# Banksylel/Restrictive-Hierarchical-Semantic-Segmentation

Measured on AMD Instinct MI355X. Metric: train images/sec (620x620, hier-HRNet-W48), higher is better.
Workload: dtype f32 (fp16x2 split on fp16 MFMA, 22-bit operands, fp32 accumulate; exact-fp32 MFMA on the small problems); 1 GPU; HRNet-W48 hierarchical (class_tree_tl.json), 620x620, batch 4 per GPU, train_epoch batch body (fwd L passes, prediction prep + metrics, CE+Dice+consistency, bwd, grad all-reduce, AdamW, metric vectors, one D2H readback of loss+metrics); global_batch=4, parallelism=dp1, launch=launch tape replay, rccl_ranks=1, level_passes=batched (one launch per layer for all L passes)

## Files before the change

restrictive-hierarchical-semantic-segmentation_amd/csrc/conv.hip:

```cpp
#include "conv_common.h"

static bool igemm_overridden() { return hrseg_g_igemm_wtm || hrseg_g_igemm_kc || hrseg_g_igemm_db || hrseg_g_igemm_ksplit; }

__global__ void zero_f32_kernel(float* __restrict__ p, size_t n) {
  for (size_t i = (size_t)blockIdx.x * blockDim.x + threadIdx.x; i < n; i += (size_t)gridDim.x * blockDim.x) p[i] = 0.f;
}
static void zero_f32(float* p, size_t n, hipStream_t st) {
  size_t blocks = (n + 255) / 256;
  if (blocks > 2048) blocks = 2048;
  hipLaunchKernelGGL(zero_f32_kernel, dim3((unsigned)blocks), dim3(256), 0, st, p, n);
}

static IgemmPlan plan_igemm(const IgemmArgs& a) {
  IgemmPlan pl;
  pl.wtn = (a.N % 48 == 0) ? 3 : (a.N % 64 == 0) ? 4 : (a.N % 32 == 0) ? 2 : 1;
  const int kc_max = (a.K % 48 == 0) ? 3 : (a.K % 32 == 0) ? 2 : 1;
  const int ntn = a.N / (16 * pl.wtn);
  const long blocks128 = (long)ceil_div(a.M, 128) * ntn;
  const bool large = blocks128 >= 384;
  pl.wtm = large ? 2 : 1;
  pl.kc = large ? 1 : kc_max;
  pl.db = 1;
  pl.ksplit = 1;
  const long blocks = (long)ceil_div(a.M, 64 * pl.wtm) * ntn;
// ... 550 lines not shown
    if (check_wgrad_span(a[i])) return 1;
    g.gx[i] = gx;
    end += gx * tiles;
    g.blk_end[i] = end;
    g.a[i] = a[i];
  }
  if (sp) {
    hrseg_count(CNT_WGRAD_SP_GROUP);
    return launch_wgrad_group_sp(g, tn, tk, end, st);
  }
  hrseg_count(CNT_WGRAD_F32_GROUP);
  return launch_wgrad_group_f32(g, tn, tk, end, st);
}

static int wgrad9_tnk(const hrseg_conv_shape_t& s) {
  if (!hrseg_g_wgrad9 || s.ksize != 3 || s.stride != 1 || sp_pieces(s.precision) == 0) return 0;
  if (s.Cin % 48 == 0 && s.Cout % 48 == 0) return 3;
  if (s.Cin % 64 == 0 && s.Cout % 64 == 0) return 4;
  return 0;
}
static const int WG9_TARGET[5] = {256, 256, 128, 128, 96};
static void wgrad9_plan(const hrseg_conv_shape_t& s, int tnk, Wgrad9Args& a, int group_n) {
  a.B = s.B; a.H = s.Hi; a.W = s.Wi; a.Cin = s.Cin; a.Cout = s.Cout; a.ldx = s.ldx; a.lddy = s.ldy;
  a.tiles_x = ceil_div(s.Wi, 16); a.tiles_y = ceil_div(s.Hi, 4);
  a.ntiles = s.B * a.tiles_x * a.tiles_y;
  const int npairs = (s.Cout / (16 * tnk)) * (s.Cin / (16 * tnk));
  const int by_n[5] = {0, hrseg_g_wgrad9_blocks1, hrseg_g_wgrad9_blocks2, hrseg_g_wgrad9_blocks3, hrseg_g_wgrad9_blocks4};
  const int target = (group_n <= 4 && by_n[group_n]) ? by_n[group_n] : hrseg_g_wgrad9_blocks ? hrseg_g_wgrad9_blocks : WG9_TARGET[group_n < 4 ? group_n : 4];
  int chunks = ceil_div(target, npairs);
  if (chunks > a.ntiles) chunks = a.ntiles;
  if (chunks < 1) chunks = 1;
  a.per = ceil_div(a.ntiles, chunks);
  a.nchunks = ceil_div(a.ntiles, a.per);
}
struct Wg9Plan { int tnk; Wgrad9Args a[WG9_MAXG]; };
static bool wgrad9_plan_all(int n, const hrseg_conv_shape_t* shapes, Wg9Plan& pl) {
  if (n < 1 || n > WG9_MAXG) return false;
  pl.tnk = wgrad9_tnk(shapes[0]);
  if (!pl.tnk) return false;
  for (int i = 0; i < n; ++i) {
    if (wgrad9_tnk(shapes[i]) != pl.tnk || shapes[i].precision != shapes[0].precision) return false;
    wgrad9_plan(shapes[i], pl.tnk, pl.a[i], n);
  }
  return true;
}
static size_t wgrad9_ws_bytes(int n, const hrseg_conv_shape_t* shapes) {
  Wg9Plan pl;
// ... 224 lines not shown
      c.Ho = hc; c.Wo = wc; c.M = s->B * hc * wc;
      c.oys = c.oxs = 2; c.oy0 = py; c.ox0 = px;
      pack_taps(c, n, oy, ox, wtp);
      cls[ncls++] = c;
    }
  if (ncls >= 2) {
    const int rc = launch_group_checked(cls, ncls, s->precision, st, "igemm_group(dgrad s2)");
    if (rc <= 0) return rc;
  }
  for (int i = 0; i < ncls; ++i) {
    if (int e = dispatch_igemm(cls[i], s->precision, st)) return e;
    HRSEG_LAUNCH_CHECK("igemm_conv(dgrad s2)");
  }
  return 0;
}

static int wgrad_one(const float* x, const float* dy, float* dw, const hrseg_conv_shape_t* s_in, hipStream_t st,
                     const char* who) {
  hrseg_conv_shape_t sh;
  resolve_wgrad_shapes(1, s_in, &sh);
  const hrseg_conv_shape_t* s = &sh;
  HRSEG_CHECK_ARG(x && dy && dw, "%s: null pointer", who);
  if (s->Cin <= HRSEG_SMALL_CIN_MAX) {
    const long M = (long)s->B * s->Ho * s->Wo;
    const int nblk_target = hrseg_g_deterministic ? 1 : hrseg_g_wgrad_blocks ? hrseg_g_wgrad_blocks : 512;
    int ppb = (int)ceil_div(ceil_div(M, nblk_target), 64) * 64;
    launch_small_cin_wgrad(x, dy, dw, s, ppb, st);
    hrseg_count(CNT_SMALL_CIN);
    HRSEG_LAUNCH_CHECK("conv_small_cin_wgrad");
    return 0;
  }
  HRSEG_CHECK_ARG(s->Cin % 16 == 0 && s->Cout % 16 == 0, "%s: channels (%d,%d) must be multiples of 16", who, s->Cin, s->Cout);
  HRSEG_CHECK_ARG(s->ldx % 4 == 0 && s->ldy % 4 == 0, "%s: ld must be a multiple of 4", who);
  WgradArgs a;
  fill_wgrad_args(a, x, dy, dw, s);
  if (const int ns = sp_pieces(s->precision)) {
    if (int e = dispatch_wgrad_sp(ns, a, st)) return e;
    HRSEG_LAUNCH_CHECK("wgrad_sp");
    return 0;
  }
  const int tn = (s->Cout % 48 == 0) ? 3 : (s->Cout % 64 == 0) ? 4 : (s->Cout % 32 == 0) ? 2 : 1;
  const int tk = (s->Cin % 48 == 0) ? 3 : (s->Cin % 64 == 0) ? 4 : (s->Cin % 32 == 0) ? 2 : 1;
  const int tiles = (a.Cout / (16 * tn)) * (a.Cin / (16 * tk)) * a.T;
  const int pix = hrseg_g_wgrad_pix ? hrseg_g_wgrad_pix : 64, db = hrseg_g_wgrad_db ? hrseg_g_wgrad_db : 1;
  const int target = hrseg_g_wgrad_blocks ? hrseg_g_wgrad_blocks : wgrad_target_blocks(tiles);
  if (int e = launch_wgrad_f32(a, tn, tk, pix, db, target, st)) return e;
  hrseg_count(CNT_WGRAD_F32);
  HRSEG_LAUNCH_CHECK("wgrad");
  return 0;
}
// ... 137 lines not shown
```

restrictive-hierarchical-semantic-segmentation_amd/csrc/conv_common.h:

```cpp
#pragma once
#include "common.h"

struct IgemmArgs {
  const float* x;
  const float* w;
  const float* bias;
  float* y;
  int ldx, ldy;
  int B, Hi, Wi, K;
  int Ho, Wo, N;
  int M;
  int sy, sx;
  int Hy, Wy, oys, oxs, oy0, ox0;
  int ntaps;
  unsigned long long offy_pk, offx_pk, wtap_pk;
  int T;
  int accumulate;
  float rcp_hw, rcp_w;
  int direct_out;
  const float* xmax;
  float wscale, wscale_inv;
  int oy_min, ox_min;
  const unsigned char* wimg;
  int cv_w1, cv_nb;
// ... 73 lines not shown
struct WeightImageGroup {
  int n;
  int ns;
  int blk_end[MAXG];
  int kind[MAXG];
  int K[MAXG];
  float wscale[MAXG];
  const float* w[MAXG];
  unsigned char* img[MAXG];
};
struct WeightImageTabEntry {
  const float* w;
  unsigned char* img;
  int K, kind, ns, blk_end;
  float wscale;
  int pad;
};

struct Wgrad9Args {
  const float* x; const float* dy; float* ws;
  const float* dymax;
  int ldx, lddy, B, H, W, Cin, Cout;
  int tiles_x, tiles_y, ntiles, nchunks, per;
  int exp_nosplit;
  int x_presplit;
};
#define WG9_MAXG 8
struct Wgrad9Group {
  int n;
  int blk_end[WG9_MAXG];
  Wgrad9Args a[WG9_MAXG];
};
struct Wgrad9Reduce {
  int n;
  int blk_end[WG9_MAXG];
  const float* ws[WG9_MAXG];
  float* dw[WG9_MAXG];
  int nchunks[WG9_MAXG];
  long n4[WG9_MAXG];
};

int launch_igemm_f32(const IgemmArgs& a, const IgemmPlan& pl, hipStream_t st);
int launch_igemm_group_f32(const IgemmGroup& g, int wtm, int wtn, int kc, hipStream_t st);
int launch_wgrad_f32(const WgradArgs& a, int tn, int tk, int pix, int db, int target, hipStream_t st);
int launch_wgrad_group_f32(const WgradGroup& g, int tn, int tk, int nblocks, hipStream_t st);
int launch_sp_kernel(int ns, const IgemmArgs& a, const SpPlan& pl, hipStream_t st);
int launch_spw_kernel(const IgemmArgs& a, int wtn, int ksplit, unsigned char* img, hipStream_t st, bool two_slab_ok);
int launch_sp_group_kernel(int ns, const IgemmGroup& g, int wtm, int wtn, bool full, hipStream_t st);
int launch_patch_sp_kernel(int ns, const IgemmArgs& a, int wtn, int cs, int flip, int blocks, int ntotal, hipStream_t st);
int launch_sp_pgroup_kernel(int ns, const IgemmGroup& g, int wtm, int wtn, int cs, int flip, hipStream_t st);
int launch_ws_kernel(const IgemmArgs& a, int kind, int flip, int blocks, int ntotal, hipStream_t st, int ns = 4);
int launch_ws_group_kernel(const IgemmGroup& g, int flip, hipStream_t st, int ns = 4);
int launch_weight_images(const WeightImageGroup& g, int nblocks, hipStream_t st);
int launch_weight_image_table(const WeightImageTabEntry* tab, int n, int nblocks, hipStream_t st);
int launch_wgrad_sp_kernel(int ns, const WgradArgs& a, int tn, int tk, int gx, int tiles, hipStream_t st);
int launch_wgrad_group_sp(const WgradGroup& g, int tn, int tk, int nblocks, hipStream_t st);
int launch_wgrad_spw_kernel(const WgradArgs& a, int nwc, int gx, int tiles, hipStream_t st);
int launch_wgrad9_kernels(int ns, int tnk, const Wgrad9Group& g, int nblocks, const Wgrad9Reduce& r, int rblocks, hipStream_t st);
int check_wgrad_span(const WgradArgs& a);
#define HRSEG_SMALL_CIN_MAX 8
void launch_small_cin_fwd(const float* x, const float* w, const float* bias, float* y, const hrseg_conv_shape_t* s, hipStream_t st);
void launch_small_cin_wgrad(const float* x, const float* dy, float* dw, const hrseg_conv_shape_t* s, int pix_per_block, hipStream_t st);
void launch_small_cin_dgrad(const float* dy, const float* w, float* dx, int accumulate, const hrseg_conv_shape_t* s, hipStream_t st);

bool scratch_usable();
unsigned char* scratch_reserve(hipStream_t st, size_t bytes);
bool ws_make_images(IgemmArgs* a, const int* kinds, int n, hipStream_t st, int ns);
```

restrictive-hierarchical-semantic-segmentation_amd/csrc/conv_small.hip:

```cpp
#include "conv_common.h"

template <int CMAX>
__global__ __launch_bounds__(256) void conv_small_cin_fwd_kernel(const float* __restrict__ x, int ldx,
                                                                 const float* __restrict__ w,
                                                                 const float* __restrict__ bias,
                                                                 float* __restrict__ y, int ldy, int B, int Hi,
                                                                 int Wi, int Cin, int Ho, int Wo, int Cout,
                                                                 int ks, int stride, const float* __restrict__ res, int ldr,
                                                                 int relu) {
  __shared__ float wl[64 * 9 * CMAX];
  const int T = ks * ks, pad = (ks - 1) / 2;
  const int cb = blockIdx.y * 64;
  for (int i = threadIdx.x; i < 64 * T * Cin; i += 256) {
    const int co = i / (T * Cin);
    wl[i] = (cb + co < Cout) ? w[(size_t)(cb + co) * T * Cin + (i - co * T * Cin)] : 0.f;
  }
  __syncthreads();
  const long M = (long)B * Ho * Wo;
  const long m = (long)blockIdx.x * 64 + (threadIdx.x & 63);
  const int cg = threadIdx.x >> 6;
  if (m >= M) return;
  const int b = (int)(m / ((long)Ho * Wo));
  const int rem = (int)(m - (long)b * Ho * Wo);
  const int oy = rem / Wo, ox = rem - oy * Wo;
// ... 44 lines not shown
    for (int kh = 0; kh < 3; ++kh) {
      const int iy = oy * stride + kh - 1;
      const bool rok = (unsigned)iy < (unsigned)Hi;
#pragma unroll
      for (int kw = 0; kw < 3; ++kw) {
        const int ix = ox * stride + kw - 1;
        const bool ok = rok & ((unsigned)ix < (unsigned)Wi);
        const float* xp = x + ((size_t)(b * Hi + (ok ? iy : 0)) * Wi + (ok ? ix : 0)) * ldx;
#pragma unroll
        for (int ci = 0; ci < 3; ++ci) {
          const float xv = ok ? xp[ci] : 0.f;
#pragma unroll
          for (int j = 0; j < 4; ++j) acc[j] = fmaf(xv, wr[(kh * 3 + kw) * 3 + ci][j], acc[j]);
        }
      }
    }
    f32x4 v = acc + bv;
    if (res) v += *reinterpret_cast<const f32x4*>(res + (size_t)m * ldr + co);
    if (relu) v = relu_nan(v);
    *reinterpret_cast<f32x4*>(y + (size_t)m * ldy + co) = v;
  }
}

__global__ __launch_bounds__(256) void conv_cin3_k3_wgrad_kernel(const float* __restrict__ x, int ldx, const float* __restrict__ dy,
                                                                 int lddy, float* __restrict__ dw, int B, int Hi, int Wi, int Ho,
                                                                 int Wo, int stride, int pix_per_block) {
  constexpr int P = 64;
  __shared__ __attribute__((aligned(16))) float dys[P][64];
  __shared__ __attribute__((aligned(16))) float xs[P][9][4];
  __shared__ float red[3][64][28];
  const int tid = threadIdx.x;
  const int co0 = blockIdx.y * 64, col = tid & 63, pg = tid >> 6;
  const int M = B * Ho * Wo, hw = Ho * Wo;
  const int lo = blockIdx.x * pix_per_block;
  const int hi = min(lo + pix_per_block, M);
  float acc[9][3];
#pragma unroll
  for (int t = 0; t < 9; ++t)
#pragma unroll
    for (int c = 0; c < 3; ++c) acc[t][c] = 0.f;
  for (int s0 = lo; s0 < hi; s0 += P) {
#pragma unroll
    for (int r = 0; r < (P * 16) / 256; ++r) {
      const int j = tid + 256 * r;
      const int pp = j >> 4, c4 = (j & 15) * 4;
      const int m = s0 + pp;
      f32x4 v = {0.f, 0.f, 0.f, 0.f};
      if (m < hi) v = *reinterpret_cast<const f32x4*>(dy + (size_t)m * lddy + co0 + c4);
      *reinterpret_cast<f32x4*>(&dys[pp][c4]) = v;
    }
    for (int j = tid; j < P * 9; j += 256) {
      const int pp = j / 9, t = j - pp * 9;
      const int m = s0 + pp;
      f32x4 v = {0.f, 0.f, 0.f, 0.f};
      if (m < hi) {
        const int b = m / hw, rem = m - b * hw;
        const int oy = rem / Wo, ox = rem - oy * Wo;
        const int iy = oy * stride + t / 3 - 1, ix = ox * stride + t % 3 - 1;
        if ((unsigned)iy < (unsigned)Hi && (unsigned)ix < (unsigned)Wi) {
          const float* xp = x + ((size_t)(b * Hi + iy) * Wi + ix) * ldx;
          v = f32x4{xp[0], xp[1], xp[2], 0.f};
        }
      }
      *reinterpret_cast<f32x4*>(&xs[pp][t][0]) = v;
    }
    __syncthreads();
#pragma unroll 4
    for (int q = 0; q < P / 4; ++q) {
      const int pp = pg * (P / 4) + q;
      const float g = dys[pp][col];
#pragma unroll
      for (int t = 0; t < 9; ++t) {
        const f32x4 xv = *reinterpret_cast<const f32x4*>(&xs[pp][t][0]);
#pragma unroll
        for (int c = 0; c < 3; ++c) acc[t][c] = fmaf(g, xv[c], acc[t][c]);
      }
    }
    __syncthreads();
  }
  if (pg > 0) {
#pragma unroll
    for (int t = 0; t < 9; ++t)
#pragma unroll
      for (int c = 0; c < 3; ++c) red[pg - 1][col][t * 3 + c] = acc[t][c];
  }
  __syncthreads();
  if (pg == 0) {
#pragma unroll
    for (int t = 0; t < 9; ++t)
#pragma unroll
      for (int c = 0; c < 3; ++c) {
        const float v = ((acc[t][c] + red[0][col][t * 3 + c]) + red[1][col][t * 3 + c]) + red[2][col][t * 3 + c];
        atomicAdd(dw + ((size_t)(co0 + col) * 9 + t) * 3 + c, v);
      }
  }
}

template <int CMAX>
__global__ __launch_bounds__(256) void conv_small_cin_wgrad_kernel(const float* __restrict__ x, int ldx,
                                                                   const float* __restrict__ dy, int lddy,
                                                                   float* __restrict__ dw, int B, int Hi,
                                                                   int Wi, int Cin, int Ho, int Wo, int Cout,
                                                                   int ks, int stride, int pix_per_block) {
  constexpr int P = 64;
  __shared__ __attribute__((aligned(16))) float dys[P][64];
  __shared__ __attribute__((aligned(16))) float xs[P][12][CMAX];
  const int T = ks * ks, pad = (ks - 1) / 2;
  const int tid = threadIdx.x;
  const int co0 = blockIdx.y * 64, co = co0 + (tid & 63);
  const int tg = tid >> 6;
  const int M = B * Ho * Wo, hw = Ho * Wo;
  const int lo = blockIdx.x * pix_per_block;
  const int hi = min(lo + pix_per_block, M);
  float acc[3][CMAX];
#pragma unroll
  for (int a = 0; a < 3; ++a)
#pragma unroll
    for (int c = 0; c < CMAX; ++c) acc[a][c] = 0.f;
// ... 103 lines not shown
  for (int c = 0; c < CMAX; ++c)
    if (c < Cin) d[c] = accumulate ? d[c] + acc[c] : acc[c];
}

void launch_small_cin_fwd(const float* x, const float* w, const float* bias, float* y, const hrseg_conv_shape_t* s, hipStream_t st) {
  const float* res = s->residual;
  const int ldr = s->ldr, relu = s->relu;
  const long M = (long)s->B * s->Ho * s->Wo;
  if (s->Cin == 3 && s->ksize == 3 && s->Cout % 64 == 0 && s->ldy % 4 == 0 && (!res || ldr % 4 == 0) && M < (1L << 31) && hrseg_g_small_cin3) {
    long gx = ceil_div(M, 16);
    if (gx > 4096) gx = 4096;
    hipLaunchKernelGGL(conv_cin3_k3_fwd_kernel, dim3((unsigned)gx, s->Cout / 64), dim3(256), 0, st, x, s->ldx, w, bias, y, s->ldy, s->B,
                       s->Hi, s->Wi, s->Ho, s->Wo, s->stride, res, ldr, relu);
    return;
  }
  dim3 grid(ceil_div(M, 64), ceil_div(s->Cout, 64));
  if (s->Cin <= 4)
    hipLaunchKernelGGL(conv_small_cin_fwd_kernel<4>, grid, dim3(256), 0, st, x, s->ldx, w, bias, y, s->ldy, s->B, s->Hi, s->Wi,
                       s->Cin, s->Ho, s->Wo, s->Cout, s->ksize, s->stride, res, ldr, relu);
  else
    hipLaunchKernelGGL(conv_small_cin_fwd_kernel<8>, grid, dim3(256), 0, st, x, s->ldx, w, bias, y, s->ldy, s->B, s->Hi, s->Wi,
                       s->Cin, s->Ho, s->Wo, s->Cout, s->ksize, s->stride, res, ldr, relu);
}
void launch_small_cin_wgrad(const float* x, const float* dy, float* dw, const hrseg_conv_shape_t* s, int ppb, hipStream_t st) {
  const long M = (long)s->B * s->Ho * s->Wo;
  if (s->Cin == 3 && s->ksize == 3 && s->Cout % 64 == 0 && s->ldy % 4 == 0 && M < (1L << 31) && hrseg_g_small_cin3) {
    hipLaunchKernelGGL(conv_cin3_k3_wgrad_kernel, dim3(ceil_div(M, ppb), s->Cout / 64), dim3(256), 0, st, x, s->ldx, dy, s->ldy, dw,
                       s->B, s->Hi, s->Wi, s->Ho, s->Wo, s->stride, ppb);
    return;
  }
  dim3 grid(ceil_div(M, ppb), ceil_div(s->Cout, 64));
  if (s->Cin <= 4)
    hipLaunchKernelGGL(conv_small_cin_wgrad_kernel<4>, grid, dim3(256), 0, st, x, s->ldx, dy, s->ldy, dw, s->B, s->Hi, s->Wi,
                       s->Cin, s->Ho, s->Wo, s->Cout, s->ksize, s->stride, ppb);
  else
    hipLaunchKernelGGL(conv_small_cin_wgrad_kernel<8>, grid, dim3(256), 0, st, x, s->ldx, dy, s->ldy, dw, s->B, s->Hi, s->Wi,
                       s->Cin, s->Ho, s->Wo, s->Cout, s->ksize, s->stride, ppb);
}
void launch_small_cin_dgrad(const float* dy, const float* w, float* dx, int accumulate, const hrseg_conv_shape_t* s, hipStream_t st) {
  const long npix = (long)s->B * s->Hi * s->Wi;
  hipLaunchKernelGGL(conv_small_cin_dgrad_kernel, dim3(ceil_div(npix, 256)), dim3(256), 0, st, dy, s->ldy, w, dx, s->ldx,
                     accumulate, s->B, s->Hi, s->Wi, s->Cin, s->Ho, s->Wo, s->Cout, s->ksize, s->stride);
}
```

restrictive-hierarchical-semantic-segmentation_amd/csrc/conv_wgrad_sp.hip:

```cpp
#include "conv_common.h"
#include "sp_arith.h"

typedef short s16x4 __attribute__((ext_vector_type(4)));
typedef short s16x8 __attribute__((ext_vector_type(8)));

__device__ __forceinline__ s16x4 sp_tr_read(const unsigned char* p) {
  return __builtin_amdgcn_ds_read_tr16_b64_v4i16((s16x4 __attribute__((address_space(3)))*)(p));
}

constexpr int sp_row_stride(int channels) {
  int s = (2 * channels + 31) / 32;
  if (s % 2 == 0) ++s;
  return 32 * s;
}

template <int NS, int TN, int TK>
struct SpWgradLds {
  static constexpr int PIX = 128;
  static constexpr int SA = sp_row_stride(16 * TN), SB = sp_row_stride(16 * TK);
  static constexpr int PIECE = PIX * (SA + SB);
  static constexpr int STAGE = sp_np(NS) * PIECE;
  static constexpr int RED = 4 * TK * 256 * 4;
  static constexpr int BYTES = (STAGE > RED) ? STAGE : RED;
};
// ... 284 lines not shown
      }
}

template <int NS, int TN, int TK, int NWR, int NWC>
__global__ __launch_bounds__(64 * NWR * NWC) void wgrad_spw_kernel(WgradArgs p) {
  __shared__ __attribute__((aligned(16))) unsigned char lds[SpWgradWideLds<NS, TN, TK, NWR, NWC>::BYTES];
  const int tiles = gridDim.y, nblk = gridDim.x * gridDim.y;
  const int r = xcd_remap(blockIdx.y * gridDim.x + blockIdx.x, nblk);
  wgrad_spw_body<NS, TN, TK, NWR, NWC>(p, lds, r / tiles, r % tiles);
}

template <int NS, int TN, int TK>
__global__ __launch_bounds__(256) void wgrad_sp_group_kernel(WgradGroup grp) {
  __shared__ __attribute__((aligned(16))) unsigned char lds[SpWgradLds<NS, TN, TK>::BYTES];
  int g = 0;
  while (g + 1 < grp.n && (int)blockIdx.x >= grp.blk_end[g]) ++g;
  const int lo = g ? grp.blk_end[g - 1] : 0;
  const int nblk = grp.blk_end[g] - lo;
  const int tiles = nblk / grp.gx[g];
  const int r = xcd_remap(blockIdx.x - lo, nblk);
  wgrad_sp_body<NS, TN, TK>(grp.a[g], lds, r / tiles, r % tiles);
}

template <int NS, int TNK>
struct SpWgrad9Lds {
  static constexpr int S = sp_row_stride(16 * TNK);
  static constexpr int DYPIX = 64, XPIX = 6 * 18;
  static constexpr int PIECE = (DYPIX + XPIX) * S;
  static constexpr int BYTES = sp_np(NS) * PIECE;
};

template <int NS, int TNK>
__device__ __forceinline__ void wgrad9_sp_body(const Wgrad9Args& p, unsigned char* lds, const int pair, const int chunk) {
  using L = SpWgrad9Lds<NS, TNK>;
  constexpr int S = L::S, PIECE = L::PIECE, XBASE = L::DYPIX * S;
  constexpr int GPP = TNK * 4;
  constexpr int NT = 192, PR = NT / GPP;
  constexpr int DY_LOADS = (L::DYPIX + PR - 1) / PR, X_LOADS = (L::XPIX + PR - 1) / PR, LOADS = DY_LOADS + X_LOADS;
  const int tid = threadIdx.x, lane = tid & 63, kh = tid >> 6;
  const int g = lane >> 4, li = lane & 15;
  const int nkt = p.Cin / (16 * TNK);
  const int ct = pair / nkt, kt = pair - ct * nkt;
  const int n0 = ct * 16 * TNK, k0 = kt * 16 * TNK;
  const int t_lo = chunk * p.per, t_hi = min(t_lo + p.per, p.ntiles);
  float dyscale, dyinv;
  sp_pow2_scale(p.dymax, dyscale, dyinv);

  f32x4 rg[LOADS];
  const int pix0 = tid / GPP, gq = tid - pix0 * GPP;
  const bool swork = pix0 < PR;
  unsigned g_rel[LOADS];
  int g_yx[LOADS];
#pragma unroll
  for (int i = 0; i < LOADS; ++i) {
    if (i < DY_LOADS) {
      const int pix = pix0 + PR * i;
      const bool ex = swork & (pix < L::DYPIX);
      g_rel[i] = ex ? ((unsigned)((pix >> 4) * p.W + (pix & 15)) * (unsigned)p.lddy + (unsigned)(n0 + 4 * gq)) * 4u : HRSEG_BUF_OOB;
      g_yx[i] = ex ? ((pix >> 4) << 8) | (pix & 15) : 0x400000;
    } else {
      const int pix = pix0 + PR * (i - DY_LOADS);
      const int py = (pix * 3641) >> 16, px = pix - py * 18;
      const bool ex = swork & (pix < L::XPIX);
      g_rel[i] = ex ? ((unsigned)(py * p.W + px) * (unsigned)p.ldx + (unsigned)(k0 + 4 * gq)) * 4u : HRSEG_BUF_OOB;
      g_yx[i] = ex ? (py << 8) | px : 0x400000;
    }
  }
  int c_tx = t_lo % p.tiles_x, c_ty = (t_lo / p.tiles_x) % p.tiles_y, c_b = (t_lo / p.tiles_x) / p.tiles_y;
  c_tx = __builtin_amdgcn_readfirstlane(c_tx); c_ty = __builtin_amdgcn_readfirstlane(c_ty); c_b = __builtin_amdgcn_readfirstlane(c_b);
  const unsigned lddy4 = (unsigned)p.lddy * 4u, ldx4 = (unsigned)p.ldx * 4u;
  auto tile_load = [&]() {
    const int y0 = c_ty * 4, x0 = c_tx * 16;
    const __amdgpu_buffer_rsrc_t rdy = make_rsrc(p.dy + (size_t)c_b * p.H * p.W * p.lddy, (size_t)p.H * p.W * p.lddy * 4);
    const __amdgpu_buffer_rsrc_t rx = make_rsrc(p.x + (size_t)c_b * p.H * p.W * p.ldx, (size_t)p.H * p.W * p.ldx * 4);
    const unsigned dyb = (unsigned)(y0 * p.W + x0) * lddy4;
    const unsigned xb = (unsigned)((y0 - 1) * p.W + x0 - 1) * ldx4;
    const bool dy_full = (y0 + 4 <= p.H) & (x0 + 16 <= p.W);
    const bool x_full = (y0 >= 1) & (x0 >= 1) & (y0 + 5 <= p.H) & (x0 + 17 <= p.W);
    if (dy_full) {
#pragma unroll
      for (int i = 0; i < DY_LOADS; ++i) rg[i] = buf_load4(rdy, g_rel[i], (int)dyb);
    } else {
#pragma unroll
      for (int i = 0; i < DY_LOADS; ++i) {
        const bool ok = (y0 + (g_yx[i] >> 8) < p.H) & (x0 + (g_yx[i] & 255) < p.W);
        rg[i] = buf_load4(rdy, ok ? g_rel[i] + dyb : HRSEG_BUF_OOB, 0);
      }
    }
    if (x_full) {
#pragma unroll
      for (int i = DY_LOADS; i < LOADS; ++i) rg[i] = buf_load4(rx, g_rel[i], (int)xb);
    } else {
#pragma unroll
      for (int i = DY_LOADS; i < LOADS; ++i) {
        const bool ok = ((unsigned)(y0 - 1 + (g_yx[i] >> 8)) < (unsigned)p.H) & ((unsigned)(x0 - 1 + (g_yx[i] & 255)) < (unsigned)p.W);
        rg[i] = buf_load4(rx, ok ? g_rel[i] + xb : HRSEG_BUF_OOB, 0);
      }
    }
    if (++c_tx == p.tiles_x) {
      c_tx = 0;
      if (++c_ty == p.tiles_y) { c_ty = 0; ++c_b; }
// ... 7 lines not shown
        const u32x4 raw = __builtin_bit_cast(u32x4, rg[i]);
#pragma unroll
        for (int s = 0; s < sp_np(NS); ++s) pc[s] = u32x2{raw[(2 * s) & 3], raw[(2 * s + 1) & 3]};
      } else {
        sp_split4<NS>(rg[i], pc, i < DY_LOADS ? dyscale : 1.f);
      }
      const int pix = (i < DY_LOADS) ? pix0 + PR * i : L::DYPIX + pix0 + PR * (i - DY_LOADS);
      const int o = pix * S + gq * 8;
      if (swork && (i < DY_LOADS ? pix < L::DYPIX : pix < L::DYPIX + L::XPIX)) {
#pragma unroll
        for (int s = 0; s < sp_np(NS); ++s) *reinterpret_cast<u32x2*>(lds + s * PIECE + o) = pc[s];
      }
    }
  };

  f32x4 acc[3][TNK][TNK];
#pragma unroll
  for (int w = 0; w < 3; ++w)
#pragma unroll
    for (int n = 0; n < TNK; ++n)
#pragma unroll
      for (int k = 0; k < TNK; ++k) acc[w][n][k] = f32x4{0.f, 0.f, 0.f, 0.f};

  const int lrow = li >> 2, lcol = (li & 3) * 8;
  const int dy_lane = (4 * g + lrow) * S + lcol;
  const int x_lane = XBASE + (kh * 18 + 4 * g + lrow) * S + lcol;

  if (t_lo < t_hi) tile_load();
  for (int t = t_lo; t < t_hi; ++t) {
    __syncthreads();
    tile_store();
    if (t + 1 < t_hi) tile_load();
    __syncthreads();
    bf16x8 afr[TNK][sp_np(NS)], bfr[TNK][sp_np(NS)];
    auto read_a = [&](int ks) {
#pragma unroll
      for (int n = 0; n < TNK; ++n)
#pragma unroll
        for (int pc = 0; pc < sp_np(NS); ++pc) {
          const s16x4 v0 = sp_tr_read(lds + pc * PIECE + dy_lane + (2 * ks) * 16 * S + n * 32);
          const s16x4 v1 = sp_tr_read(lds + pc * PIECE + dy_lane + (2 * ks + 1) * 16 * S + n * 32);
          afr[n][pc] = __builtin_bit_cast(bf16x8, (s16x8){v0[0], v0[1], v0[2], v0[3], v1[0], v1[1], v1[2], v1[3]});
        }
    };
    auto read_b = [&](int grp, int k) {
      const int ks = grp / 3, kw = grp % 3;
#pragma unroll
      for (int pc = 0; pc < sp_np(NS); ++pc) {
        const s16x4 v0 = sp_tr_read(lds + pc * PIECE + x_lane + ((2 * ks) * 18 + kw) * S + k * 32);
        const s16x4 v1 = sp_tr_read(lds + pc * PIECE + x_lane + ((2 * ks + 1) * 18 + kw) * S + k * 32);
        bfr[k][pc] = __builtin_bit_cast(bf16x8, (s16x8){v0[0], v0[1], v0[2], v0[3], v1[0], v1[1], v1[2], v1[3]});
      }
    };
    read_a(0);
#pragma unroll
    for (int k = 0; k < TNK; ++k) read_b(0, k);
#pragma unroll
    for (int grp = 0; grp < 6; ++grp) {
      const int kw = grp % 3;
      if (grp == 3) read_a(1);
#pragma unroll
      for (int k = 0; k < TNK; ++k) {
#pragma unroll
        for (int pr = 0; pr < sp_nprod(NS); ++pr)
#pragma unroll
          for (int n = 0; n < TNK; ++n) acc[kw][n][k] = sp_mma_p<NS>(pr, afr[n], bfr[k], acc[kw][n][k]);
        __builtin_amdgcn_sched_barrier(0);
        if (grp + 1 < 6) read_b(grp + 1, k);
        __builtin_amdgcn_sched_barrier(0);
      }
    }
  }

  float* out = p.ws + (size_t)chunk * p.Cout * 9 * p.Cin;
  const int row9 = 9 * p.Cin;
  const int obase = ((n0 + 4 * g) * 9 + kh * 3) * p.Cin + k0 + li;
#pragma unroll
  for (int kw = 0; kw < 3; ++kw)
#pragma unroll
    for (int n = 0; n < TNK; ++n)
#pragma unroll
      for (int k = 0; k < TNK; ++k)
#pragma unroll
        for (int e = 0; e < 4; ++e)
          out[obase + (16 * n + e) * row9 + kw * p.Cin + 16 * k] = NS == 4 ? acc[kw][n][k][e] * dyinv : acc[kw][n][k][e];
}

template <int NS, int TNK>
__device__ __forceinline__ void wgrad9_sp_group_entry(const Wgrad9Group& grp, unsigned char* lds) {
  const int bid = (int)blockIdx.x;
  int gi = 0;
  while (gi + 1 < grp.n && bid >= grp.blk_end[gi]) ++gi;
  const int local = bid - (gi ? grp.blk_end[gi - 1] : 0);
  const Wgrad9Args& p = grp.a[gi];
  const int npairs = (p.Cout / (16 * TNK)) * (p.Cin / (16 * TNK));
  wgrad9_sp_body<NS, TNK>(p, lds, local % npairs, local / npairs);
}
template <int NS>
__global__ __launch_bounds__(192) __attribute__((amdgpu_waves_per_eu(2, 2))) void wgrad9_sp_group_kernel3(Wgrad9Group grp) {
  __shared__ __attribute__((aligned(16))) unsigned char lds[SpWgrad9Lds<NS, 3>::BYTES];
  wgrad9_sp_group_entry<NS, 3>(grp, lds);
}
template <int NS>
__global__ __launch_bounds__(192) void wgrad9_sp_group_kernel4(Wgrad9Group grp) {
  __shared__ __attribute__((aligned(16))) unsigned char lds[SpWgrad9Lds<NS, 4>::BYTES];
  wgrad9_sp_group_entry<NS, 4>(grp, lds);
}

__global__ __launch_bounds__(256) void wgrad9_reduce_kernel(Wgrad9Reduce r) {
  __shared__ f32x4 part[8][32];
  int gi = 0;
  while (gi + 1 < r.n && (int)blockIdx.x >= r.blk_end[gi]) ++gi;
  const int lo = gi ? r.blk_end[gi - 1] : 0;
  const long n4 = r.n4[gi];
  const f32x4* ws = reinterpret_cast<const f32x4*>(r.ws[gi]);
  f32x4* dw = reinterpret_cast<f32x4*>(r.dw[gi]);
  const int nch = r.nchunks[gi];
  const int e = threadIdx.x & 31, j = threadIdx.x >> 5;
  for (long i0 = (long)(blockIdx.x - lo) * 32; i0 < n4; i0 += (long)(r.blk_end[gi] - lo) * 32) {
    const long i = i0 + e;
    f32x4 s = {0.f, 0.f, 0.f, 0.f};
    if (i < n4)
      for (int c = j; c < nch; c += 8) s += ws[(size_t)c * n4 + i];
    part[j][e] = s;
    __syncthreads();
    if (j == 0 && i < n4)
      dw[i] += ((part[0][e] + part[1][e]) + (part[2][e] + part[3][e])) + ((part[4][e] + part[5][e]) + (part[6][e] + part[7][e]));
    __syncthreads();
  }
// ... 4 lines not shown
#define WS(TN_, TK_) if (tn == TN_ && tk == TK_) { hipLaunchKernelGGL((wgrad_sp_kernel<NS, TN_, TK_>), dim3(gx, tiles), dim3(256), 0, st, a); return 0; }
  WS(1, 1) WS(1, 2) WS(1, 3) WS(1, 4) WS(2, 1) WS(2, 2) WS(2, 3) WS(2, 4)
  WS(3, 1) WS(3, 2) WS(3, 3) WS(3, 4) WS(4, 1) WS(4, 2) WS(4, 3) WS(4, 4)
  if constexpr (NS == 4) { WS(5, 5) }
#undef WS
  return HRSEG_ERR_UNSUPPORTED;
}
int launch_wgrad_sp_kernel(int ns, const WgradArgs& a, int tn, int tk, int gx, int tiles, hipStream_t st) {
  return ns == 4 ? launch_wgrad_sp<4>(a, tn, tk, gx, tiles, st) : ns == 3 ? launch_wgrad_sp<3>(a, tn, tk, gx, tiles, st)
       : ns == 2 ? launch_wgrad_sp<2>(a, tn, tk, gx, tiles, st) : launch_wgrad_sp<1>(a, tn, tk, gx, tiles, st);
}
int launch_wgrad_spw_kernel(const WgradArgs& a, int nwc, int gx, int tiles, hipStream_t st) {
  if (nwc == 3) hipLaunchKernelGGL((wgrad_spw_kernel<4, 5, 3, 3, 3>), dim3(gx, tiles), dim3(576), 0, st, a);
  else hipLaunchKernelGGL((wgrad_spw_kernel<4, 5, 3, 3, 1>), dim3(gx, tiles), dim3(192), 0, st, a);
  return 0;
}
int launch_wgrad_group_sp(const WgradGroup& g, int tn, int tk, int nblocks, hipStream_t st) {
#define WGS(TN_, TK_) if (tn == TN_ && tk == TK_) { hipLaunchKernelGGL((wgrad_sp_group_kernel<4, TN_, TK_>), dim3(nblocks), dim3(256), 0, st, g); return 0; }
  WGS(3, 3) WGS(3, 4) WGS(4, 3) WGS(4, 4)
#undef WGS
  return 1;
}
int launch_wgrad9_kernels(int ns, int tnk, const Wgrad9Group& g, int nblocks, const Wgrad9Reduce& r, int rblocks, hipStream_t st) {
#define W9(NS_) if (ns == NS_) { \
    if (tnk == 3) hipLaunchKernelGGL((wgrad9_sp_group_kernel3<NS_>), dim3(nblocks), dim3(192), 0, st, g); \
    else hipLaunchKernelGGL((wgrad9_sp_group_kernel4<NS_>), dim3(nblocks), dim3(192), 0, st, g); }
  W9(1) W9(2) W9(3) W9(4)
#undef W9
  HRSEG_LAUNCH_CHECK("wgrad9");
  hipLaunchKernelGGL(wgrad9_reduce_kernel, dim3(rblocks), dim3(256), 0, st, r);
  HRSEG_LAUNCH_CHECK("wgrad9_reduce");
  return 0;
}
```

restrictive-hierarchical-semantic-segmentation_amd/csrc/runtime.h:

```cpp
#pragma once

#define HRSEG_FAMILIES(X)                   \
  X(WS, "ws", 1)                            \
  X(WS_GROUP, "ws_group", 1)                \
  X(PATCH_SP, "patch_sp", 1)                \
  X(SP_IM2COL, "sp_im2col", 1)              \
  X(SP_PGROUP, "sp_pgroup", 1)              \
  X(SP_GROUP, "sp_group", 1)                \
  X(F32, "f32", 1)                          \
  X(F32_GROUP, "f32_group", 1)              \
  X(WGRAD_SP, "wgrad_sp", 1)                \
  X(WGRAD_F32, "wgrad_f32", 1)              \
  X(WGRAD_F32_GROUP, "wgrad_f32_group", 1)  \
  X(WGRAD9, "wgrad9", 1)                    \
  X(SMALL_CIN, "small_cin", 1)              \
  X(SP_WIDE, "sp_wide", 1)                  \
  X(WS_CANVAS, "ws_canvas", 0)              \
  X(WGRAD_SP_GROUP, "wgrad_sp_group", 1)    \
  X(WGRAD_SP_T5, "wgrad_sp_t5", 0)          \
  X(WGRAD_SP_WIDE, "wgrad_sp_wide", 1)      \
  X(AUG_IMAGE, "augment_image", 0)          \
  X(AUG_TARGETS, "augment_targets", 0)      \
  X(DECODE_LABELS, "decode_labels", 0)      \
  X(SCORE_LABELS, "score_labels", 0)        \
// ... 28 lines not shown
  X(wgrad_group_max, 0, 0, "  ... its upper clamp (automatic: 2048)")                                                                \
  X(sp_wtm, 0, 0, "split-precision plan: pixel tiles per wave")                                                                      \
  X(sp_wtn, 0, 0, "split-precision plan: channel tile in 16-channel units; set, it keeps every problem off the wave-specialised body") \
  X(sp_ksplit, 0, 0, "split-precision plan: split-K factor")                                                                         \
  X(sp_patch, 1, 0, "0 = never use the halo-patch body")                                                                             \
  X(sp_persist, 2, 0, "persistent patch blocks per CU (0 = one tile per block)")                                                     \
  X(sp_ws, 1, 0, "0 = never use the wave-specialised body")                                                                          \
  X(sp_ws_waste, 200, 0, "wave-specialised body: tile padding accepted, percent of the image")                                       \
  X(small_cin3, 1, 0, "0 = the 3-channel 3x3 first layer stays on the generic Cin <= 8 kernels (conv_small.hip)")                    \
  X(sp_ws_bf16, 1, 0, "0 = the bf16 arithmetic (one piece, one product) stays off the wave-specialised kernels")                     \
  X(sp_ws_n48, 1, 0, "0 = 48-channel tilings stay on the block-synchronous kernels")                                                 \
  X(sp_img, 1, 0, "0 = the block-synchronous patch body splits its weights on the fly")                                              \
  X(wgrad9, 1, 0, "0 = never use the nine-tap weight-gradient kernel")                                                               \
  X(ws_epi_early, 1, 0, "0 = the wave-specialised body reads accumulate / residual values at the tile's end")                        \
  X(exp_nosplit_x, 0, 0, "MEASUREMENT ONLY -- the ceiling of 'activations pre-split in HBM' (results wrong)")                        \
  X(x_split, 1, 0, "0 = hrseg_conv_x_split_ok always answers no (activations stay fp32 everywhere)")                                 \
  X(ws_epi_cost, 0, 0, "grouped wave-specialised launch: a tile's epilogue in slab times (0 = default, negative = none; conv.hip)")   \
  X(ws_epi_acc_cost, 0, 0, "  ... of an accumulating / residual epilogue")                                                           \
  X(wgrad9_blocks, 0, 0, "nine-tap weight gradient: target blocks per problem (0 = the table in conv.hip)")                          \
  X(wgrad9_blocks1, 0, 0, "  ... for a call of one problem")                                                                         \
  X(wgrad9_blocks2, 0, 0, "  ... of two")                                                                                            \
  X(wgrad9_blocks3, 0, 0, "  ... of three")                                                                                          \
  X(wgrad9_blocks4, 0, 0, "  ... of four")                                                                                           \
  X(sp_wide, 1, 0, "0 = never use the wide-tile im2col body, 2 = also on short reductions (tests)")                                  \
  X(sp_ws_canvas, 5, 0, "canvas tiling of small images: least cut of the padded area, percent (0 = per-image tiles everywhere)")     \
  X(wgrad_group_sp, 1, 0, "0 = grouped tap-per-block weight gradients stay on the fp32 kernel")                                      \
  X(wgrad_sp_t5, 1, 0, "0 = no 80 x 80 tiles in the tap-per-block weight gradient")                                                  \
  X(wgrad_sp_wide, 1, 0, "0 = never the wide-tile weight-gradient body")                                                             \
  X(sp_wide_min_blocks, 256, 0, "wide-tile im2col body: least number of 128-pixel blocks")                                           \
  X(sp_patch_min_tiles, 192, 1, "routing threshold: least tile count of the halo-patch body")                                        \
  X(auto_min_pixels, 8192, 1, "routing threshold: HRSEG_CONV_AUTO runs fp16x2 from this many output pixels on")                      \
  X(sp_ws_min_tiles, 96, 1, "routing threshold: least tile count of the wave-specialised body")                                      \
  X(deterministic, 0, 0, "1 = every float reduction with a run-dependent order takes its single-adder form (common.h)")             \
  X(bwd_multi_slab, 0, 0, "multi-target bilinear transpose: channels of a slab of the streaming body (0 = automatic, < 0 = the gather body)") \
  X(bwd_multi_bands, 0, 0, "  ... its bands of target rows per image (0 = automatic; clamped to the coarsest target's rows)")        \
  X(fuse_bwd_multi, 1, 0, "0 = the fuse layers' backward transposes each low-resolution term in a launch of its own (engine.py)")
#define HRSEG_X(key, def, restore, meaning) extern int hrseg_g_##key;
HRSEG_KNOBS(HRSEG_X)
#undef HRSEG_X
```

Before: 97.05 images/s.

## Add 8x8 pixel tiles to nine-tap wgrad and rewrite Cin3 stem wgrad kernel

```diff
diff --git a/restrictive-hierarchical-semantic-segmentation_amd/csrc/conv.hip b/restrictive-hierarchical-semantic-segmentation_amd/csrc/conv.hip
--- a/restrictive-hierarchical-semantic-segmentation_amd/csrc/conv.hip
+++ b/restrictive-hierarchical-semantic-segmentation_amd/csrc/conv.hip
@@ -596,7 +596,9 @@
 static const int WG9_TARGET[5] = {256, 256, 128, 128, 96};
 static void wgrad9_plan(const hrseg_conv_shape_t& s, int tnk, Wgrad9Args& a, int group_n) {
   a.B = s.B; a.H = s.Hi; a.W = s.Wi; a.Cin = s.Cin; a.Cout = s.Cout; a.ldx = s.ldx; a.lddy = s.ldy;
-  a.tiles_x = ceil_div(s.Wi, 16); a.tiles_y = ceil_div(s.Hi, 4);
+  const int t16 = ceil_div(s.Wi, 16) * ceil_div(s.Hi, 4), t8 = ceil_div(s.Wi, 8) * ceil_div(s.Hi, 8);
+  a.tw = hrseg_g_wgrad9_tile == 8 ? 8 : hrseg_g_wgrad9_tile == 16 ? 16 : t8 < t16 ? 8 : 16;
+  a.tiles_x = ceil_div(s.Wi, a.tw); a.tiles_y = ceil_div(s.Hi, 64 / a.tw);
   a.ntiles = s.B * a.tiles_x * a.tiles_y;
   const int npairs = (s.Cout / (16 * tnk)) * (s.Cin / (16 * tnk));
   const int by_n[5] = {0, hrseg_g_wgrad9_blocks1, hrseg_g_wgrad9_blocks2, hrseg_g_wgrad9_blocks3, hrseg_g_wgrad9_blocks4};
@@ -867,10 +869,7 @@
   const hrseg_conv_shape_t* s = &sh;
   HRSEG_CHECK_ARG(x && dy && dw, "%s: null pointer", who);
   if (s->Cin <= HRSEG_SMALL_CIN_MAX) {
-    const long M = (long)s->B * s->Ho * s->Wo;
-    const int nblk_target = hrseg_g_deterministic ? 1 : hrseg_g_wgrad_blocks ? hrseg_g_wgrad_blocks : 512;
-    int ppb = (int)ceil_div(ceil_div(M, nblk_target), 64) * 64;
-    launch_small_cin_wgrad(x, dy, dw, s, ppb, st);
+    launch_small_cin_wgrad(x, dy, dw, s, hrseg_g_deterministic ? 1 : hrseg_g_wgrad_blocks, st);
     hrseg_count(CNT_SMALL_CIN);
     HRSEG_LAUNCH_CHECK("conv_small_cin_wgrad");
     return 0;
diff --git a/restrictive-hierarchical-semantic-segmentation_amd/csrc/conv_common.h b/restrictive-hierarchical-semantic-segmentation_amd/csrc/conv_common.h
--- a/restrictive-hierarchical-semantic-segmentation_amd/csrc/conv_common.h
+++ b/restrictive-hierarchical-semantic-segmentation_amd/csrc/conv_common.h
@@ -119,6 +119,7 @@
   const float* dymax;
   int ldx, lddy, B, H, W, Cin, Cout;
   int tiles_x, tiles_y, ntiles, nchunks, per;
+  int tw;
   int exp_nosplit;
   int x_presplit;
 };
@@ -157,7 +158,7 @@
 int check_wgrad_span(const WgradArgs& a);
 #define HRSEG_SMALL_CIN_MAX 8
 void launch_small_cin_fwd(const float* x, const float* w, const float* bias, float* y, const hrseg_conv_shape_t* s, hipStream_t st);
-void launch_small_cin_wgrad(const float* x, const float* dy, float* dw, const hrseg_conv_shape_t* s, int pix_per_block, hipStream_t st);
+void launch_small_cin_wgrad(const float* x, const float* dy, float* dw, const hrseg_conv_shape_t* s, int nblk, hipStream_t st);
 void launch_small_cin_dgrad(const float* dy, const float* w, float* dx, int accumulate, const hrseg_conv_shape_t* s, hipStream_t st);
 
 bool scratch_usable();
diff --git a/restrictive-hierarchical-semantic-segmentation_amd/csrc/conv_small.hip b/restrictive-hierarchical-semantic-segmentation_amd/csrc/conv_small.hip
--- a/restrictive-hierarchical-semantic-segmentation_amd/csrc/conv_small.hip
+++ b/restrictive-hierarchical-semantic-segmentation_amd/csrc/conv_small.hip
@@ -90,78 +90,78 @@
   }
 }
 
+constexpr int CIN3_WG_U = 8;
 __global__ __launch_bounds__(256) void conv_cin3_k3_wgrad_kernel(const float* __restrict__ x, int ldx, const float* __restrict__ dy,
                                                                  int lddy, float* __restrict__ dw, int B, int Hi, int Wi, int Ho,
                                                                  int Wo, int stride, int pix_per_block) {
-  constexpr int P = 64;
-  __shared__ __attribute__((aligned(16))) float dys[P][64];
-  __shared__ __attribute__((aligned(16))) float xs[P][9][4];
-  __shared__ float red[3][64][28];
-  const int tid = threadIdx.x;
-  const int co0 = blockIdx.y * 64, col = tid & 63, pg = tid >> 6;
+  constexpr int U = CIN3_WG_U;
+  __shared__ float red[4][64 * 27];
+  __shared__ __attribute__((aligned(16))) float xs[4][U][28];
+  const int tid = threadIdx.x, lane = tid & 63;
+  const int wave = __builtin_amdgcn_readfirstlane(tid >> 6);
+  const int co0 = blockIdx.y * 64;
   const int M = B * Ho * Wo, hw = Ho * Wo;
   const int lo = blockIdx.x * pix_per_block;
   const int hi = min(lo + pix_per_block, M);
-  float acc[9][3];
-#pragma unroll
-  for (int t = 0; t < 9; ++t)
-#pragma unroll
-    for (int c = 0; c < 3; ++c) acc[t][c] = 0.f;
-  for (int s0 = lo; s0 < hi; s0 += P) {
-#pragma unroll
-    for (int r = 0; r < (P * 16) / 256; ++r) {
-      const int j = tid + 256 * r;
-      const int pp = j >> 4, c4 = (j & 15) * 4;
-      const int m = s0 + pp;
-      f32x4 v = {0.f, 0.f, 0.f, 0.f};
-      if (m < hi) v = *reinterpret_cast<const f32x4*>(dy + (size_t)m * lddy + co0 + c4);
-      *reinterpret_cast<f32x4*>(&dys[pp][c4]) = v;
-    }
-    for (int j = tid; j < P * 9; j += 256) {
-      const int pp = j / 9, t = j - pp * 9;
-      const int m = s0 + pp;
-      f32x4 v = {0.f, 0.f, 0.f, 0.f};
-      if (m < hi) {
-        const int b = m / hw, rem = m - b * hw;
-        const int oy = rem / Wo, ox = rem - oy * Wo;
-        const int iy = oy * stride + t / 3 - 1, ix = ox * stride + t % 3 - 1;
-        if ((unsigned)iy < (unsigned)Hi && (unsigned)ix < (unsigned)Wi) {
-          const float* xp = x + ((size_t)(b * Hi + iy) * Wi + ix) * ldx;
-          v = f32x4{xp[0], xp[1], xp[2], 0.f};
-        }
-      }
-      *reinterpret_cast<f32x4*>(&xs[pp][t][0]) = v;
-    }
-    __syncthreads();
-#pragma unroll 4
-    for (int q = 0; q < P / 4; ++q) {
-      const int pp = pg * (P / 4) + q;
-      const float g = dys[pp][col];
-#pragma unroll
-      for (int t = 0; t < 9; ++t) {
-        const f32x4 xv = *reinterpret_cast<const f32x4*>(&xs[pp][t][0]);
-#pragma unroll
-        for (int c = 0; c < 3; ++c) acc[t][c] = fmaf(g, xv[c], acc[t][c]);
-      }
-    }
-    __syncthreads();
-  }
-  if (pg > 0) {
-#pragma unroll
-    for (int t = 0; t < 9; ++t)
-#pragma unroll
-      for (int c = 0; c < 3; ++c) red[pg - 1][col][t * 3 + c] = acc[t][c];
-  }
+  const bool small = M < (1 << 24);
+  const float rcp_hw = small ? 1.0f / (float)hw : 0.f, rcp_w = small ? 1.0f / (float)Wo : 0.f;
+  const int half = lane < 27 ? 0 : 1, k = lane < 54 ? lane - 27 * half : 0;
+  const int kh = k / 9, kw = (k / 3) % 3, c = k % 3;
+  const float* dyp = dy + co0 + lane;
+  auto load_dy = [&](int m0, float (&g)[U]) {
+#pragma unroll
+    for (int u = 0; u < U; ++u) g[u] = dyp[(size_t)min(m0 + u, M - 1) * lddy];
+  };
+  auto load_x = [&](int m0, float (&xv)[U / 2], bool (&ok)[U / 2]) {
+#pragma unroll
+    for (int j = 0; j < U / 2; ++j) {
+      const int m = m0 + 2 * j + half, mc = min(m, M - 1);
+      const int b = fdiv(mc, hw, rcp_hw), rem = mc - b * hw;
+      const int oy = fdiv(rem, Wo, rcp_w), ox = rem - oy * Wo;
+      const int iy = oy * stride + kh - 1, ix = ox * stride + kw - 1;
+      ok[j] = (lane < 54) & (m < hi) & ((unsigned)iy < (unsigned)Hi) & ((unsigned)ix < (unsigned)Wi);
+      xv[j] = x[((size_t)(b * Hi + min(max(iy, 0), Hi - 1)) * Wi + min(max(ix, 0), Wi - 1)) * ldx + c];
+    }
+  };
+  float acc[27];
+#pragma unroll
+  for (int i = 0; i < 27; ++i) acc[i] = 0.f;
+  float g[U], gn[U], xv[U / 2], xn[U / 2];
+  bool okn[U / 2];
+  int m0 = lo + wave * U;
+  if (m0 < hi) {
+    load_dy(m0, gn);
+    load_x(m0, xn, okn);
+  }
+  for (; m0 < hi; m0 += 4 * U) {
+#pragma unroll
+    for (int u = 0; u < U; ++u) g[u] = (m0 + u < hi) ? gn[u] : 0.f;
+#pragma unroll
+    for (int j = 0; j < U / 2; ++j) xv[j] = okn[j] ? xn[j] : 0.f;
+    load_dy(m0 + 4 * U, gn);
+    load_x(m0 + 4 * U, xn, okn);
+    __builtin_amdgcn_fence(__ATOMIC_RELEASE, "wavefront");
+    __builtin_amdgcn_wave_barrier();
+    if (lane < 54) {
+#pragma unroll
+      for (int j = 0; j < U / 2; ++j) xs[wave][2 * j + half][k] = xv[j];
+    }
+    __builtin_amdgcn_fence(__ATOMIC_ACQ_REL, "wavefront");
+    __builtin_amdgcn_wave_barrier();
+#pragma unroll
+    for (int u = 0; u < U; ++u) {
+      f32x4 s[7];
+#pragma unroll
+      for (int i = 0; i < 7; ++i) s[i] = *reinterpret_cast<const f32x4*>(&xs[wave][u][4 * i]);
+#pragma unroll
+      for (int i = 0; i < 27; ++i) acc[i] = fmaf(g[u], s[i >> 2][i & 3], acc[i]);
+    }
+  }
+#pragma unroll
+  for (int i = 0; i < 27; ++i) red[wave][lane * 27 + i] = acc[i];
   __syncthreads();
-  if (pg == 0) {
-#pragma unroll
-    for (int t = 0; t < 9; ++t)
-#pragma unroll
-      for (int c = 0; c < 3; ++c) {
-        const float v = ((acc[t][c] + red[0][col][t * 3 + c]) + red[1][col][t * 3 + c]) + red[2][col][t * 3 + c];
-        atomicAdd(dw + ((size_t)(co0 + col) * 9 + t) * 3 + c, v);
-      }
-  }
+  for (int i = tid; i < 64 * 27; i += 256)
+    atomicAdd(dw + (size_t)co0 * 27 + i, ((red[0][i] + red[1][i]) + red[2][i]) + red[3][i]);
 }
 
 template <int CMAX>
@@ -311,13 +311,16 @@
     hipLaunchKernelGGL(conv_small_cin_fwd_kernel<8>, grid, dim3(256), 0, st, x, s->ldx, w, bias, y, s->ldy, s->B, s->Hi, s->Wi,
                        s->Cin, s->Ho, s->Wo, s->Cout, s->ksize, s->stride, res, ldr, relu);
 }
-void launch_small_cin_wgrad(const float* x, const float* dy, float* dw, const hrseg_conv_shape_t* s, int ppb, hipStream_t st) {
+void launch_small_cin_wgrad(const float* x, const float* dy, float* dw, const hrseg_conv_shape_t* s, int nblk, hipStream_t st) {
   const long M = (long)s->B * s->Ho * s->Wo;
   if (s->Cin == 3 && s->ksize == 3 && s->Cout % 64 == 0 && s->ldy % 4 == 0 && M < (1L << 31) && hrseg_g_small_cin3) {
+    if (!nblk) nblk = 512;
+    const int ppb = (int)ceil_div(ceil_div(M, nblk), 4 * CIN3_WG_U) * 4 * CIN3_WG_U;
     hipLaunchKernelGGL(conv_cin3_k3_wgrad_kernel, dim3(ceil_div(M, ppb), s->Cout / 64), dim3(256), 0, st, x, s->ldx, dy, s->ldy, dw,
                        s->B, s->Hi, s->Wi, s->Ho, s->Wo, s->stride, ppb);
     return;
   }
+  const int ppb = (int)ceil_div(ceil_div(M, nblk ? nblk : 512), 64) * 64;
   dim3 grid(ceil_div(M, ppb), ceil_div(s->Cout, 64));
   if (s->Cin <= 4)
     hipLaunchKernelGGL(conv_small_cin_wgrad_kernel<4>, grid, dim3(256), 0, st, x, s->ldx, dy, s->ldy, dw, s->B, s->Hi, s->Wi,
diff --git a/restrictive-hierarchical-semantic-segmentation_amd/csrc/conv_wgrad_sp.hip b/restrictive-hierarchical-semantic-segmentation_amd/csrc/conv_wgrad_sp.hip
--- a/restrictive-hierarchical-semantic-segmentation_amd/csrc/conv_wgrad_sp.hip
+++ b/restrictive-hierarchical-semantic-segmentation_amd/csrc/conv_wgrad_sp.hip
@@ -330,18 +330,21 @@
   wgrad_sp_body<NS, TN, TK>(grp.a[g], lds, r / tiles, r % tiles);
 }
 
-template <int NS, int TNK>
+template <int NS, int TNK, int TW = 16>
 struct SpWgrad9Lds {
   static constexpr int S = sp_row_stride(16 * TNK);
-  static constexpr int DYPIX = 64, XPIX = 6 * 18;
+  static constexpr int TH = 64 / TW, PW = TW + 2;
+  static constexpr int DYPIX = 64, XPIX = (TH + 2) * PW;
   static constexpr int PIECE = (DYPIX + XPIX) * S;
   static constexpr int BYTES = sp_np(NS) * PIECE;
 };
 
-template <int NS, int TNK>
+template <int NS, int TNK, int TW>
 __device__ __forceinline__ void wgrad9_sp_body(const Wgrad9Args& p, unsigned char* lds, const int pair, const int chunk) {
-  using L = SpWgrad9Lds<NS, TNK>;
+  static_assert(TW == 16 || TW == 8, "tile width");
+  using L = SpWgrad9Lds<NS, TNK, TW>;
   constexpr int S = L::S, PIECE = L::PIECE, XBASE = L::DYPIX * S;
+  constexpr int TH = L::TH, PW = L::PW, TWS = TW == 16 ? 4 : 3;
   constexpr int GPP = TNK * 4;
   constexpr int NT = 192, PR = NT / GPP;
   constexpr int DY_LOADS = (L::DYPIX + PR - 1) / PR, X_LOADS = (L::XPIX + PR - 1) / PR, LOADS = DY_LOADS + X_LOADS;
@@ -364,11 +367,11 @@
     if (i < DY_LOADS) {
       const int pix = pix0 + PR * i;
       const bool ex = swork & (pix < L::DYPIX);
-      g_rel[i] = ex ? ((unsigned)((pix >> 4) * p.W + (pix & 15)) * (unsigned)p.lddy + (unsigned)(n0 + 4 * gq)) * 4u : HRSEG_BUF_OOB;
-      g_yx[i] = ex ? ((pix >> 4) << 8) | (pix & 15) : 0x400000;
+      g_rel[i] = ex ? ((unsigned)((pix >> TWS) * p.W + (pix & (TW - 1))) * (unsigned)p.lddy + (unsigned)(n0 + 4 * gq)) * 4u : HRSEG_BUF_OOB;
+      g_yx[i] = ex ? ((pix >> TWS) << 8) | (pix & (TW - 1)) : 0x400000;
     } else {
       const int pix = pix0 + PR * (i - DY_LOADS);
-      const int py = (pix * 3641) >> 16, px = pix - py * 18;
+      const int py = (pix * (TW == 16 ? 3641 : 6554)) >> 16, px = pix - py * PW;
       const bool ex = swork & (pix < L::XPIX);
       g_rel[i] = ex ? ((unsigned)(py * p.W + px) * (unsigned)p.ldx + (unsigned)(k0 + 4 * gq)) * 4u : HRSEG_BUF_OOB;
       g_yx[i] = ex ? (py << 8) | px : 0x400000;
@@ -378,13 +381,13 @@
   c_tx = __builtin_amdgcn_readfirstlane(c_tx); c_ty = __builtin_amdgcn_readfirstlane(c_ty); c_b = __builtin_amdgcn_readfirstlane(c_b);
   const unsigned lddy4 = (unsigned)p.lddy * 4u, ldx4 = (unsigned)p.ldx * 4u;
   auto tile_load = [&]() {
-    const int y0 = c_ty * 4, x0 = c_tx * 16;
+    const int y0 = c_ty * TH, x0 = c_tx * TW;
     const __amdgpu_buffer_rsrc_t rdy = make_rsrc(p.dy + (size_t)c_b * p.H * p.W * p.lddy, (size_t)p.H * p.W * p.lddy * 4);
     const __amdgpu_buffer_rsrc_t rx = make_rsrc(p.x + (size_t)c_b * p.H * p.W * p.ldx, (size_t)p.H * p.W * p.ldx * 4);
     const unsigned dyb = (unsigned)(y0 * p.W + x0) * lddy4;
     const unsigned xb = (unsigned)((y0 - 1) * p.W + x0 - 1) * ldx4;
-    const bool dy_full = (y0 + 4 <= p.H) & (x0 + 16 <= p.W);
-    const bool x_full = (y0 >= 1) & (x0 >= 1) & (y0 + 5 <= p.H) & (x0 + 17 <= p.W);
+    const bool dy_full = (y0 + TH <= p.H) & (x0 + TW <= p.W);
+    const bool x_full = (y0 >= 1) & (x0 >= 1) & (y0 + TH + 1 <= p.H) & (x0 + TW + 1 <= p.W);
     if (dy_full) {
 #pragma unroll
       for (int i = 0; i < DY_LOADS; ++i) rg[i] = buf_load4(rdy, g_rel[i], (int)dyb);
@@ -438,9 +441,10 @@
 #pragma unroll
       for (int k = 0; k < TNK; ++k) acc[w][n][k] = f32x4{0.f, 0.f, 0.f, 0.f};
 
+  constexpr int XSTEP = TW == 16 ? PW : 2 * PW;
   const int lrow = li >> 2, lcol = (li & 3) * 8;
   const int dy_lane = (4 * g + lrow) * S + lcol;
-  const int x_lane = XBASE + (kh * 18 + 4 * g + lrow) * S + lcol;
+  const int x_lane = XBASE + (TW == 16 ? kh * PW + 4 * g + lrow : (kh + (g >> 1)) * PW + 4 * (g & 1) + lrow) * S + lcol;
 
   if (t_lo < t_hi) tile_load();
   for (int t = t_lo; t < t_hi; ++t) {
@@ -463,8 +467,8 @@
       const int ks = grp / 3, kw = grp % 3;
 #pragma unroll
       for (int pc = 0; pc < sp_np(NS); ++pc) {
-        const s16x4 v0 = sp_tr_read(lds + pc * PIECE + x_lane + ((2 * ks) * 18 + kw) * S + k * 32);
-        const s16x4 v1 = sp_tr_read(lds + pc * PIECE + x_lane + ((2 * ks + 1) * 18 + kw) * S + k * 32);
+        const s16x4 v0 = sp_tr_read(lds + pc * PIECE + x_lane + ((2 * ks) * XSTEP + kw) * S + k * 32);
+        const s16x4 v1 = sp_tr_read(lds + pc * PIECE + x_lane + ((2 * ks + 1) * XSTEP + kw) * S + k * 32);
         bfr[k][pc] = __builtin_bit_cast(bf16x8, (s16x8){v0[0], v0[1], v0[2], v0[3], v1[0], v1[1], v1[2], v1[3]});
       }
     };
@@ -502,7 +506,7 @@
           out[obase + (16 * n + e) * row9 + kw * p.Cin + 16 * k] = NS == 4 ? acc[kw][n][k][e] * dyinv : acc[kw][n][k][e];
 }
 
-template <int NS, int TNK>
+template <int NS, int TNK, int TWM>
 __device__ __forceinline__ void wgrad9_sp_group_entry(const Wgrad9Group& grp, unsigned char* lds) {
   const int bid = (int)blockIdx.x;
   int gi = 0;
@@ -510,17 +514,18 @@
   const int local = bid - (gi ? grp.blk_end[gi - 1] : 0);
   const Wgrad9Args& p = grp.a[gi];
   const int npairs = (p.Cout / (16 * TNK)) * (p.Cin / (16 * TNK));
-  wgrad9_sp_body<NS, TNK>(p, lds, local % npairs, local / npairs);
-}
-template <int NS>
+  if (TWM == 8 || (TWM == 0 && p.tw == 8)) wgrad9_sp_body<NS, TNK, 8>(p, lds, local % npairs, local / npairs);
+  else wgrad9_sp_body<NS, TNK, 16>(p, lds, local % npairs, local / npairs);
+}
+template <int NS, int TWM = 16>
 __global__ __launch_bounds__(192) __attribute__((amdgpu_waves_per_eu(2, 2))) void wgrad9_sp_group_kernel3(Wgrad9Group grp) {
   __shared__ __attribute__((aligned(16))) unsigned char lds[SpWgrad9Lds<NS, 3>::BYTES];
-  wgrad9_sp_group_entry<NS, 3>(grp, lds);
-}
-template <int NS>
+  wgrad9_sp_group_entry<NS, 3, TWM>(grp, lds);
+}
+template <int NS, int TWM = 16>
 __global__ __launch_bounds__(192) void wgrad9_sp_group_kernel4(Wgrad9Group grp) {
   __shared__ __attribute__((aligned(16))) unsigned char lds[SpWgrad9Lds<NS, 4>::BYTES];
-  wgrad9_sp_group_entry<NS, 4>(grp, lds);
+  wgrad9_sp_group_entry<NS, 4, TWM>(grp, lds);
 }
 
 __global__ __launch_bounds__(256) void wgrad9_reduce_kernel(Wgrad9Reduce r) {
@@ -571,10 +576,13 @@
   return 1;
 }
 int launch_wgrad9_kernels(int ns, int tnk, const Wgrad9Group& g, int nblocks, const Wgrad9Reduce& r, int rblocks, hipStream_t st) {
-#define W9(NS_) if (ns == NS_) { \
-    if (tnk == 3) hipLaunchKernelGGL((wgrad9_sp_group_kernel3<NS_>), dim3(nblocks), dim3(192), 0, st, g); \
-    else hipLaunchKernelGGL((wgrad9_sp_group_kernel4<NS_>), dim3(nblocks), dim3(192), 0, st, g); }
-  W9(1) W9(2) W9(3) W9(4)
+  int twm = g.a[0].tw;
+  for (int i = 1; i < g.n; ++i)
+    if (g.a[i].tw != twm) twm = 0;
+#define W9(NS_, TWM_) if (ns == NS_ && twm == TWM_) { \
+    if (tnk == 3) hipLaunchKernelGGL((wgrad9_sp_group_kernel3<NS_, TWM_>), dim3(nblocks), dim3(192), 0, st, g); \
+    else hipLaunchKernelGGL((wgrad9_sp_group_kernel4<NS_, TWM_>), dim3(nblocks), dim3(192), 0, st, g); }
+  W9(1, 16) W9(2, 16) W9(3, 16) W9(4, 16) W9(1, 8) W9(2, 8) W9(3, 8) W9(4, 8) W9(1, 0) W9(2, 0) W9(3, 0) W9(4, 0)
 #undef W9
   HRSEG_LAUNCH_CHECK("wgrad9");
   hipLaunchKernelGGL(wgrad9_reduce_kernel, dim3(rblocks), dim3(256), 0, st, r);
diff --git a/restrictive-hierarchical-semantic-segmentation_amd/csrc/runtime.h b/restrictive-hierarchical-semantic-segmentation_amd/csrc/runtime.h
--- a/restrictive-hierarchical-semantic-segmentation_amd/csrc/runtime.h
+++ b/restrictive-hierarchical-semantic-segmentation_amd/csrc/runtime.h
@@ -74,6 +74,7 @@
   X(wgrad9_blocks2, 0, 0, "  ... of two")                                                                                            \
   X(wgrad9_blocks3, 0, 0, "  ... of three")                                                                                          \
   X(wgrad9_blocks4, 0, 0, "  ... of four")                                                                                           \
+  X(wgrad9_tile, 0, 0, "nine-tap weight gradient: pixel-tile width, 16 = 4 x 16, 8 = 8 x 8 (0 = fewer tiles per image, conv.hip)")  \
   X(sp_wide, 1, 0, "0 = never use the wide-tile im2col body, 2 = also on short reductions (tests)")                                  \
   X(sp_ws_canvas, 5, 0, "canvas tiling of small images: least cut of the padded area, percent (0 = per-image tiles everywhere)")     \
   X(wgrad_group_sp, 1, 0, "0 = grouped tap-per-block weight gradients stay on the fp32 kernel")                                      \
```

New measurement: 97.93 images/s, median of 6. No clear change (+0.9%).
